# mcap91/SpatialCore

Measured on AMD Instinct MI355X. Metric: genes/sec Moran's I (1000 perms, 1M cells, k=15), higher is better.
Workload: dtype f64

## Files before the change

spatialcore_amd/csrc/sc_moran.hip:

```cpp
#include <math.h>
#include <stdlib.h>

#include <functional>
#include <vector>

#include "sc_permgen.h"


#define MP_PERMS_PER_BLOCK 32

__global__ __launch_bounds__(256) void k_moran_perm(const double *__restrict__ Zt,
                                                    const double *__restrict__ Lt,
                                                    const int32_t *__restrict__ perm,
                                                    double *__restrict__ partial, int64_t n,
                                                    int64_t pstride, int n_perm, int64_t cells_per_split)
{
    const int wave = threadIdx.x >> 6, lane = threadIdx.x & 63;
    const int r = lane >> 3, q = lane & 7;
    const int pbase = blockIdx.y * MP_PERMS_PER_BLOCK + wave * 8;
    if (pbase >= n_perm) return;
    const int p = pbase + r;
    const int pc = p < n_perm ? p : n_perm - 1;
    const int64_t c0 = (int64_t)blockIdx.x * cells_per_split;
    int64_t c1 = c0 + cells_per_split;
// ... 22 lines not shown
        const double2 z4 = Z2[(i + 4) * 8];
        const double2 z5 = Z2[(i + 5) * 8];
        const double2 z6 = Z2[(i + 6) * 8];
        const double2 z7 = Z2[(i + 7) * 8];
        a0x = fma(z0.x, l0.x, a0x); a0y = fma(z0.y, l0.y, a0y);
        a1x = fma(z1.x, l1.x, a1x); a1y = fma(z1.y, l1.y, a1y);
        a0x = fma(z2.x, l2.x, a0x); a0y = fma(z2.y, l2.y, a0y);
        a1x = fma(z3.x, l3.x, a1x); a1y = fma(z3.y, l3.y, a1y);
        a0x = fma(z4.x, l4.x, a0x); a0y = fma(z4.y, l4.y, a0y);
        a1x = fma(z5.x, l5.x, a1x); a1y = fma(z5.y, l5.y, a1y);
        a0x = fma(z6.x, l6.x, a0x); a0y = fma(z6.y, l6.y, a0y);
        a1x = fma(z7.x, l7.x, a1x); a1y = fma(z7.y, l7.y, a1y);
    }
    for (; i < c1; ++i) {
        const double2 l = L2[(int64_t)prow[i] * 8];
        const double2 z = Z2[i * 8];
        a0x = fma(z.x, l.x, a0x);
        a0y = fma(z.y, l.y, a0y);
    }
    if (p < n_perm) {
        double2 *out = reinterpret_cast<double2 *>(partial) +
                       ((int64_t)blockIdx.x * n_perm + p) * 8 + q;
        *out = make_double2(a0x + a1x, a0y + a1y);
    }
}

__global__ __launch_bounds__(256) void k_moran_finalize(const double *__restrict__ partial,
                                                        const double *__restrict__ seff, const double *__restrict__ corr,
                                                        double *__restrict__ sims, double *__restrict__ raw, int n_perm, int splits,
                                                        int64_t n_genes, int64_t g0, int64_t p0)
{
    int t = blockIdx.x * blockDim.x + threadIdx.x;
    int p = t >> 4, slot = t & 15;
    if (p >= n_perm || g0 + slot >= n_genes) return;
    double s = 0.0;
    for (int k = 0; k < splits; ++k) s += partial[((int64_t)k * n_perm + p) * SC_TILE + slot];
    raw[(p0 + p) * n_genes + g0 + slot] = s;
    sims[(p0 + p) * n_genes + g0 + slot] = seff[g0 + slot] * (s - corr[g0 + slot]);
}

__global__ void k_moran_scale(const double *__restrict__ z2, const double *__restrict__ inum, const double *__restrict__ slag,
                              const double *__restrict__ mean, const double *__restrict__ lat, double *__restrict__ seff,
                              double *__restrict__ corr, double *__restrict__ thr, double *__restrict__ I, double n_over_s0,
                              double w, int64_t total)
{
    int64_t g = (int64_t)blockIdx.x * blockDim.x + threadIdx.x;
    if (g >= total) return;
    const bool l = lat[g] != 0.0;
    const double sc = l ? (n_over_s0 / z2[g]) * w : n_over_s0 / z2[g];
    const double co = l ? mean[g] * slag[g] : 0.0;
    const double v = sc * (inum[g] - co);
    seff[g] = sc;
    corr[g] = co;
    I[g] = v;
    thr[g] = l ? inum[g] : v;
}

__global__ __launch_bounds__(256) void k_moran_count(const double *__restrict__ sims, const double *__restrict__ raw,
                                                     const double *__restrict__ thr, const double *__restrict__ lat,
                                                     const double *__restrict__ z2, int n_perm,
                                                     int64_t n_genes, long long *__restrict__ count,
                                                     double *__restrict__ ssum, double *__restrict__ ssq)
{
    __shared__ double sh_a[256], sh_b[256];
    __shared__ int sh_c[256];
    int64_t g = blockIdx.x;
    const double t = thr[g];
    const bool l = lat[g] != 0.0, alive = z2[g] > 0.0;
    double a = 0.0, b = 0.0;
    int cnt = 0;
    for (int p = threadIdx.x; p < n_perm; p += 256) {
        double v = sims[(int64_t)p * n_genes + g];
        const double cv = l ? raw[(int64_t)p * n_genes + g] : v;
        cnt += (alive && cv >= t) ? 1 : 0;
        a += v;
        b += v * v;
    }
    sh_a[threadIdx.x] = a;
    sh_b[threadIdx.x] = b;
    sh_c[threadIdx.x] = cnt;
    __syncthreads();
    for (int s = 128; s > 0; s >>= 1) {
        if ((int)threadIdx.x < s) {
            sh_a[threadIdx.x] += sh_a[threadIdx.x + s];
            sh_b[threadIdx.x] += sh_b[threadIdx.x + s];
            sh_c[threadIdx.x] += sh_c[threadIdx.x + s];
        }
        __syncthreads();
    }
    if (threadIdx.x == 0) {
        count[g] = sh_c[0];
        ssum[g] = sh_a[0];
        ssq[g] = sh_b[0];
    }
}


__global__ void k_moran_centres(const double *__restrict__ mean, const double *__restrict__ lat, double *__restrict__ centre,
                                int64_t total)
{
    const int64_t g = (int64_t)blockIdx.x * blockDim.x + threadIdx.x;
    if (g < total) centre[g] = lat[g] != 0.0 ? 0.0 : mean[g];
}


#define SCORE_WAVES 16
#define SCORE_PRIVATE_WAVES 8

__device__ __forceinline__ double2 lag16_to_double2(uint32_t v) { return make_double2((double)(v & 0xffffu), (double)(v >> 16)); }


template <bool BIG>
__device__ __forceinline__ uint4 score_row(const char *const &Xg, const uint32_t &qoff, int32_t i)
{
    if constexpr (BIG) return *reinterpret_cast<const uint4 *>(Xg + ((uint64_t)(uint32_t)i * 128u + qoff));
    else return *reinterpret_cast<const uint4 *>(Xg + ((uint32_t)i * 128u + qoff));
}

template <int CB>
__device__ __forceinline__ void score_load_idx(int4 (&id)[CB / 4], const int32_t *const &irow, const int64_t &c0, int64_t b, const int64_t &nblk)
{
    const int64_t bb = b < nblk ? b : nblk - 1;
#pragma unroll
    for (int k = 0; k < CB / 4; ++k) id[k] = *reinterpret_cast<const int4 *>(irow + c0 + bb * CB + 4 * k);
}

template <int CB, bool BIG>
__device__ __forceinline__ void score_gather(uint4 (&x)[CB], const int4 (&id)[CB / 4], const char *const &Xg, const uint32_t &qoff)
{
#pragma unroll
    for (int k = 0; k < CB / 4; ++k) {
        x[4 * k + 0] = score_row<BIG>(Xg, qoff, id[k].x);
        x[4 * k + 1] = score_row<BIG>(Xg, qoff, id[k].y);
        x[4 * k + 2] = score_row<BIG>(Xg, qoff, id[k].z);
        x[4 * k + 3] = score_row<BIG>(Xg, qoff, id[k].w);
    }
}

template <int BITS, bool CENTER>
__device__ __forceinline__ void score_fma(const uint32_t (&w)[4], int t, double2 l, const double (&m)[2], double (&acc)[2])
{
    double v0, v1;
    if (BITS == 8) {
        const uint32_t h = w[t >> 1] >> (16 * (t & 1));
        v0 = (double)(h & 0xffu); v1 = (double)((h >> 8) & 0xffu);
    } else if (BITS == 16) { v0 = (double)(w[t] & 0xffffu); v1 = (double)(w[t] >> 16); }
    else if (BITS == 32) { v0 = (double)__uint_as_float(w[2 * t]); v1 = (double)__uint_as_float(w[2 * t + 1]); }
    else { v0 = __hiloint2double((int)w[1], (int)w[0]); v1 = __hiloint2double((int)w[3], (int)w[2]); }
    if constexpr (CENTER) { v0 -= m[0]; v1 -= m[1]; }
    acc[0] = fma(l.x, v0, acc[0]);
    acc[1] = fma(l.y, v1, acc[1]);
}

template <int BITS, int CB, bool BIG, bool L16 = false>
__global__ __launch_bounds__(SCORE_PRIVATE_WAVES * 64) void k_moran_score(
    const uint4 *__restrict__ narrow, const double *__restrict__ Lag, int64_t tile_elems, int tiles16,
    const double *__restrict__ mean, const int32_t *__restrict__ inv, double *__restrict__ partial, int64_t n,
    int64_t pstride, int n_perm, int64_t cells_per_split, int n_splits, int n_groups)
{
    static_assert((BITS == 8 || BITS == 16 || BITS == 32 || BITS == 64) && (CB == 4 || CB == 8), "source width / block size");
    static_assert(!L16 || BITS == 8, "16-bit lag rows belong to the uint8 source");
    constexpr int TG = BITS == 8 ? 8 : BITS == 16 ? 4 : BITS == 32 ? 2 : 1;
    constexpr bool CENTER = BITS == 16 || BITS == 32;
    constexpr int ROW = TG * 8;
    static_assert((CB * ROW) % 64 == 0, "a block's lag rows are loaded by whole wavefront instructions");
    constexpr int NI = CB / 4;
    constexpr int NL = CB * ROW / 64;
    constexpr int CSTEP = 64 / ROW;
    __shared__ double2 lds_lag[SCORE_PRIVATE_WAVES][2][CB * ROW];
    const int wave = threadIdx.x >> 6, lane = threadIdx.x & 63;
    const int r = lane >> 3, q = lane & 7;
    const int lcell0 = lane / ROW, ltile = (lane % ROW) >> 3;
    double2 *lw = &lds_lag[wave][0][0];
    const int pgroups = (n_perm + 7) >> 3;
    const int64_t n_tasks = (int64_t)n_groups * n_splits * pgroups;
    const int64_t worker = (int64_t)blockIdx.x * SCORE_PRIVATE_WAVES + wave, workers = (int64_t)gridDim.x * SCORE_PRIVATE_WAVES;

    for (int64_t task = worker; task < n_tasks; task += workers) {
        const int pg = (int)(task % pgroups);
        const int64_t rest = task / pgroups;
        const int split = (int)(rest % n_splits), grp = (int)(rest / n_splits);
        const int p = pg * 8 + r;
        const int pc = p < n_perm ? p : n_perm - 1;
        const int64_t c0 = (int64_t)split * cells_per_split;
        int64_t c1 = c0 + cells_per_split;
        if (c1 > n) c1 = n;
        const int32_t *irow = inv + (int64_t)pc * pstride;
        const char *Xg = reinterpret_cast<const char *>(narrow + (int64_t)grp * n * 8);
        const uint32_t qoff = (uint32_t)q * 16u;
        const int tiles_left = tiles16 - TG * grp;
        const double *lag_g = Lag + (int64_t)TG * grp * tile_elems;
        const double2 *lsrc = reinterpret_cast<const double2 *>(lag_g + (int64_t)(ltile < tiles_left ? ltile : 0) * tile_elems) + (lane & 7);
        const uint32_t *lag16_g = reinterpret_cast<const uint32_t *>(Lag) + (int64_t)grp * n * ROW;
        const uint32_t *lsrc16 = lag16_g + (lane % ROW);
        double m[CENTER ? TG : 1][2], acc[TG][2];
#pragma unroll
        for (int t = 0; t < TG; ++t) {
            if constexpr (CENTER) {
                const double *mt = mean + (int64_t)(TG * grp + (t < tiles_left ? t : 0)) * SC_TILE + 2 * q;
                m[t][0] = mt[0]; m[t][1] = mt[1];
            }
            acc[t][0] = acc[t][1] = 0.0;
        }
        const int64_t nblk = (c1 - c0) / CB;

        int4 ida[NI], idb[NI];
        double2 lg0, lg1, lg2, lg3;
        uint32_t lh0 = 0, lh1 = 0, lh2 = 0, lh3 = 0;
        uint4 xa[CB], xb[CB];

        auto load_idx = [&](int4 (&id)[NI], int64_t b) { score_load_idx<CB>(id, irow, c0, b, nblk); };
        auto load_lag = [&](int64_t b) {
            const int64_t bb = b < nblk ? b : nblk - 1;
            const int64_t row0 = c0 + bb * CB + lcell0;
            if constexpr (L16) {
                lh0 = lsrc16[row0 * ROW];
                if constexpr (NL > 1) lh1 = lsrc16[(row0 + CSTEP) * ROW];
                if constexpr (NL > 2) { lh2 = lsrc16[(row0 + 2 * CSTEP) * ROW]; lh3 = lsrc16[(row0 + 3 * CSTEP) * ROW]; }
            } else {
                lg0 = lsrc[row0 * 8];
                if constexpr (NL > 1) lg1 = lsrc[(row0 + CSTEP) * 8];
                if constexpr (NL > 2) { lg2 = lsrc[(row0 + 2 * CSTEP) * 8]; lg3 = lsrc[(row0 + 3 * CSTEP) * 8]; }
            }
        };
        auto gather = [&](uint4 (&x)[CB], const int4 (&id)[NI]) { score_gather<CB, BIG>(x, id, Xg, qoff); };
        auto park_lag = [&](int buf) {
            double2 *dst = lw + buf * (CB * ROW) + lane;
            if constexpr (L16) {
                dst[0] = lag16_to_double2(lh0);
                if constexpr (NL > 1) dst[64] = lag16_to_double2(lh1);
                if constexpr (NL > 2) { dst[128] = lag16_to_double2(lh2); dst[192] = lag16_to_double2(lh3); }
            } else {
                dst[0] = lg0;
                if constexpr (NL > 1) dst[64] = lg1;
                if constexpr (NL > 2) { dst[128] = lg2; dst[192] = lg3; }
            }
        };
        auto mul_cell = [&](const uint4 &x, const double2 *lr) {
            const uint32_t w[4] = {x.x, x.y, x.z, x.w};
#pragma unroll
            for (int t = 0; t < TG; ++t) score_fma<BITS, CENTER>(w, t, lr[t * 8], m[CENTER ? t : 0], acc[t]);
        };
        auto multiply = [&](const uint4 (&x)[CB], int buf) {
            const double2 *lr = lw + buf * (CB * ROW) + q;
#pragma unroll
            for (int c = 0; c < CB; ++c) mul_cell(x[c], lr + c * ROW);
        };
        auto stage = [&](const uint4 (&cur)[CB], uint4 (&nxt)[CB], int4 (&id_next)[NI], int64_t b) {
            load_lag(b + 1);
            __builtin_amdgcn_sched_barrier(0);
            gather(nxt, id_next);
            __builtin_amdgcn_sched_barrier(0);
            load_idx(id_next, b + 3);
            __builtin_amdgcn_sched_barrier(0);
            park_lag((int)((b + 1) & 1));
            multiply(cur, (int)(b & 1));
            __builtin_amdgcn_sched_barrier(0);
        };

        if (nblk > 0) {
            load_idx(ida, 0);
            load_lag(0);
            gather(xa, ida);
            load_idx(idb, 1);
            load_idx(ida, 2);
            park_lag(0);
            int64_t b = 0;
            for (; b + 2 <= nblk; b += 2) {
                stage(xa, xb, idb, b);
                stage(xb, xa, ida, b + 1);
            }
            if (b < nblk) stage(xa, xb, idb, b);
        }
        for (int64_t j = c0 + nblk * CB; j < c1; ++j) {
            const uint4 x = score_row<BIG>(Xg, qoff, irow[j]);
            const uint32_t w[4] = {x.x, x.y, x.z, x.w};
#pragma unroll
            for (int t = 0; t < TG; ++t) {
                double2 l;
                if constexpr (L16) l = lag16_to_double2(lag16_g[j * ROW + t * 8 + q]);
                else l = reinterpret_cast<const double2 *>(lag_g + (int64_t)(t < tiles_left ? t : 0) * tile_elems)[j * 8 + q];
                score_fma<BITS, CENTER>(w, t, l, m[CENTER ? t : 0], acc[t]);
            }
        }
        if (p < n_perm) {
            double2 *out = reinterpret_cast<double2 *>(partial) + (((int64_t)grp * n_splits + split) * n_perm + p) * ROW + q;
#pragma unroll
            for (int t = 0; t < TG; ++t) out[t * 8] = make_double2(acc[t][0], acc[t][1]);
        }
    }
}

#define SCORE_SB 16
#define SCORE_WG_MIN_PERMS 24

template <int BITS, int CB, bool BIG, bool L16 = false>
__global__ __launch_bounds__(SCORE_WAVES * 64) void k_moran_score_wg(
    const uint4 *__restrict__ narrow, const double *__restrict__ Lag, int64_t tile_elems, int tiles16,
    const double *__restrict__ mean, const int32_t *__restrict__ inv, double *__restrict__ partial, int64_t n,
    int64_t pstride, int n_perm, int64_t cells_per_split, int n_splits, int n_groups)
{
    static_assert((BITS == 4 || BITS == 8 || BITS == 16 || BITS == 32 || BITS == 64) && (CB == 4 || CB == 8), "source width / block size");
    constexpr bool NIB = BITS == 4;
    constexpr int TG = BITS == 8 ? 8 : BITS == 16 ? 4 : BITS == 32 ? 2 : NIB ? 4 : 1;
    constexpr bool CENTER = BITS == 16 || BITS == 32;
    constexpr int ROW = TG * 8;
    constexpr int NI = CB / 4;
    constexpr int SPS = SCORE_SB / CB;
    constexpr int PIECES = SCORE_SB * ROW;
    static_assert(PIECES <= SCORE_WAVES * 64 && (SCORE_WAVES * 64) % PIECES == 0, "every thread loads one piece");
    __shared__ double2 lds_lag[2][PIECES];
    const int wave = threadIdx.x >> 6, lane = threadIdx.x & 63;
    const int r = lane >> 3, q = lane & 7;
    const int pid = (int)threadIdx.x % PIECES;
    const int lcell = pid / ROW, ltile = (pid % ROW) >> 3;
    const int pchunks = (n_perm + 8 * SCORE_WAVES - 1) / (8 * SCORE_WAVES);
    const int64_t n_tasks = (int64_t)n_groups * n_splits * pchunks;

    for (int64_t task = blockIdx.x; task < n_tasks; task += gridDim.x) {
        const int pch = (int)(task % pchunks);
        const int64_t rest = task / pchunks;
        const int split = (int)(rest % n_splits), grp = (int)(rest / n_splits);
        const int pbase = (pch * SCORE_WAVES + (BITS != 64 ? __builtin_amdgcn_readfirstlane(wave) : wave)) * 8;
        const bool live = pbase < n_perm;
        const int p = pbase + r;
        const int pc = p < n_perm ? p : n_perm - 1;
        const int64_t c0 = (int64_t)split * cells_per_split;
        int64_t c1 = c0 + cells_per_split;
        if (c1 > n) c1 = n;
        const int32_t *irow = inv + (int64_t)pc * pstride;
        const char *Xg = reinterpret_cast<const char *>(narrow + (int64_t)grp * n * 8);
        const uint32_t qoff = (uint32_t)q * 16u;
        const int tiles_left = tiles16 - TG * grp;
        const double *lag_g = Lag + (int64_t)TG * grp * tile_elems;
        const double2 *lsrc = NIB ? reinterpret_cast<const double2 *>(Lag) + (int64_t)grp * n * ROW + (pid % ROW)
                                  : reinterpret_cast<const double2 *>(lag_g + (int64_t)(ltile < tiles_left ? ltile : 0) * tile_elems) + (pid & 7);
        constexpr int LSTRIDE = NIB ? ROW : 8;
        const uint32_t *lag16_g = reinterpret_cast<const uint32_t *>(Lag) + (int64_t)grp * n * ROW;
        const uint32_t *lsrc16 = lag16_g + (pid % ROW);
        double m[CENTER ? TG : 1][2], acc[TG][2];
#pragma unroll
        for (int t = 0; t < TG; ++t) {
            if constexpr (CENTER) {
                const double *mt = mean + (int64_t)(TG * grp + (t < tiles_left ? t : 0)) * SC_TILE + 2 * q;
                m[t][0] = mt[0]; m[t][1] = mt[1];
            }
            acc[t][0] = acc[t][1] = 0.0;
        }
        uint32_t ai[NIB ? 32 : 1];
#pragma unroll
        for (int k2 = 0; k2 < (NIB ? 32 : 1); ++k2) ai[k2] = 0u;
        const int64_t nsb = (c1 - c0) / SCORE_SB;
        const int64_t nblk = nsb * SPS;

        double2 lg;
        uint32_t lh = 0;
        uint4 xa[CB], xb[CB];
        auto park = [&](int buf) {
            if constexpr (L16) lds_lag[buf][pid] = lag16_to_double2(lh);
            else lds_lag[buf][pid] = lg;
        };

        auto load_idx = [&](int4 (&id)[NI], int64_t b) { score_load_idx<CB>(id, irow, c0, b, nblk); };
        auto load_lag = [&](int64_t sb) {
            const int64_t ss = sb < nsb ? sb : nsb - 1;
            if constexpr (L16) lh = lsrc16[(c0 + ss * SCORE_SB + lcell) * ROW];
            else lg = lsrc[(c0 + ss * SCORE_SB + lcell) * LSTRIDE];
        };
        auto gather = [&](uint4 (&x)[CB], const int4 (&id)[NI]) { score_gather<CB, BIG>(x, id, Xg, qoff); };
        auto mul_cell = [&](const uint4 &x, const double2 *lr) {
            const uint32_t w[4] = {x.x, x.y, x.z, x.w};
            if constexpr (NIB) {
#pragma unroll
                for (int t = 0; t < 4; ++t) {
                    const uint4 sp = *reinterpret_cast<const uint4 *>(&lr[t * 8]);
                    const uint32_t sw[4] = {sp.x, sp.y, sp.z, sp.w};
#pragma unroll
                    for (int e = 0; e < 8; ++e)
                        ai[t * 8 + e] += __umul24((w[t] >> (4 * e)) & 15u, (sw[e >> 1] >> (16 * (e & 1))) & 0xffffu);
                }
                return;
            }
#pragma unroll
            for (int t = 0; t < TG; ++t) score_fma<BITS, CENTER>(w, t, lr[t * 8], m[CENTER ? t : 0], acc[t]);
        };
        auto stage = [&](const uint4 (&cur)[CB], uint4 (&nxt)[CB], int4 (&id_next)[NI], int64_t sb, int k) {
            if (k == 0) load_lag(sb + 1);
            __builtin_amdgcn_sched_barrier(0);
            gather(nxt, id_next);
            __builtin_amdgcn_sched_barrier(0);
            load_idx(id_next, sb * SPS + k + 1 + SPS);
            __builtin_amdgcn_sched_barrier(0);
            const double2 *lr = &lds_lag[sb & 1][k * CB * ROW + q];
#pragma unroll
            for (int c = 0; c < CB; ++c) {
                mul_cell(cur[c], lr + c * ROW);
                if constexpr (NIB) __builtin_amdgcn_sched_barrier(0);
            }
            __builtin_amdgcn_sched_barrier(0);
            if (k == SPS - 1) {
                park((int)((sb + 1) & 1));
                __syncthreads();
            }
        };

        if (BITS != 64 && nsb > 0 && !live) {
            load_lag(0);
            park(0);
            __syncthreads();
            for (int64_t sb = 0; sb < nsb; ++sb) {
                load_lag(sb + 1);
                park((int)((sb + 1) & 1));
                __syncthreads();
            }
        } else if (nsb > 0) {
            int4 id0[NI], id1[NI], id2[NI], id3[NI];
            load_lag(0);
            load_idx(id3, 0);
            gather(xa, id3);
            load_idx(id0, 1);
            load_idx(id1, 2);
            if constexpr (SPS == 4) { load_idx(id2, 3); load_idx(id3, 4); }
            park(0);
            __syncthreads();
            for (int64_t sb = 0; sb < nsb; ++sb) {
                stage(xa, xb, id0, sb, 0);
                stage(xb, xa, id1, sb, 1);
                if constexpr (SPS == 4) {
                    stage(xa, xb, id2, sb, 2);
                    stage(xb, xa, id3, sb, 3);
                }
            }
        }
        if (live) {
            for (int64_t j = c0 + nsb * SCORE_SB; j < c1; ++j) {
                const uint4 x = score_row<BIG>(Xg, qoff, irow[j]);
                const uint32_t w[4] = {x.x, x.y, x.z, x.w};
                if constexpr (NIB) {
                    const uint4 *srow = reinterpret_cast<const uint4 *>(Lag) + ((int64_t)grp * n + j) * ROW + q;
#pragma unroll
                    for (int t = 0; t < 4; ++t) {
                        const uint4 sp = srow[t * 8];
                        const uint32_t sw[4] = {sp.x, sp.y, sp.z, sp.w};
#pragma unroll
                        for (int e = 0; e < 8; ++e)
                            ai[t * 8 + e] += __umul24((w[t] >> (4 * e)) & 15u, (sw[e >> 1] >> (16 * (e & 1))) & 0xffffu);
                    }
                    continue;
                }
#pragma unroll
                for (int t = 0; t < TG; ++t) {
                    double2 l;
                    if constexpr (L16) l = lag16_to_double2(lag16_g[j * ROW + t * 8 + q]);
                    else l = reinterpret_cast<const double2 *>(lag_g + (int64_t)(t < tiles_left ? t : 0) * tile_elems)[j * 8 + q];
                    score_fma<BITS, CENTER>(w, t, l, m[CENTER ? t : 0], acc[t]);
                }
            }
            if (p < n_perm) {
                if constexpr (NIB) {
                    double2 *out = reinterpret_cast<double2 *>(partial + ((((int64_t)grp * n_splits + split) * n_perm + p) * 256 + q * 8));
#pragma unroll
                    for (int t = 0; t < 4; ++t)
#pragma unroll
                        for (int e2 = 0; e2 < 4; ++e2)
                            out[t * 32 + e2] = make_double2((double)ai[t * 8 + 2 * e2], (double)ai[t * 8 + 2 * e2 + 1]);
                } else {
                double2 *out = reinterpret_cast<double2 *>(partial) + (((int64_t)grp * n_splits + split) * n_perm + p) * ROW + q;
#pragma unroll
                for (int t = 0; t < TG; ++t) out[t * 8] = make_double2(acc[t][0], acc[t][1]);
                }
            }
        }
    }
}

template <int GP>
__global__ __launch_bounds__(256) void k_moran_finalize_groups(const double *__restrict__ partial,
                                                               const double *__restrict__ seff,
                                                               const double *__restrict__ corr,
                                                               double *__restrict__ sims, double *__restrict__ raw, int n_perm,
                                                               int splits, int64_t n_genes, int64_t p0)
{
    const int t = blockIdx.x * blockDim.x + threadIdx.x;
    const int p = t / GP, slot = t % GP;
    const int64_t g = GP * (int64_t)blockIdx.y + slot;
    if (p >= n_perm || g >= n_genes) return;
    const double *pt = partial + (int64_t)blockIdx.y * splits * n_perm * GP;
    double s = 0.0;
    for (int k = 0; k < splits; ++k) s += pt[((int64_t)k * n_perm + p) * GP + slot];
    raw[(p0 + p) * n_genes + g] = s;
    sims[(p0 + p) * n_genes + g] = seff[g] * (s - corr[g]);
}

static int64_t score_cells_per_split(int64_t n)
{
    int64_t cps = align_up64(ceil_div64(n, 512), 8);
    return cps < 2048 ? 2048 : cps;
}

static int pick_splits(int64_t n, int n_perm_tiles, int64_t *cells_per_split)
{
    int64_t want = ceil_div64(2048, n_perm_tiles > 0 ? n_perm_tiles : 1);
    if (want < 1) want = 1;
    if (want > 256) want = 256;
    int64_t cps = align_up64(ceil_div64(n, want), 8);
    if (cps < 2048) cps = 2048;
    *cells_per_split = cps;
    return (int)ceil_div64(n, cps);
}

static int moran_check(sc_ctx *c, int64_t n_perm, const double *I_out)
{
    SC_REQUIRE(c && I_out, SC_ERR_INVALID, "sc_moran: null pointer");
    SC_REQUIRE(n_perm >= 0 && n_perm <= (1 << 24), SC_ERR_INVALID, "sc_moran: n_perm=%lld out of range",
               (long long)n_perm);
    SC_HIP(hipSetDevice(c->device));
    SC_REQUIRE(c->e_n > 0, SC_ERR_STATE, "sc_moran: no expression loaded");
    SC_REQUIRE(c->g_n > 0, SC_ERR_STATE, "sc_moran: no graph set");
    SC_REQUIRE(c->g_n == c->e_n, SC_ERR_INVALID, "sc_moran: graph has %lld rows but expression has %lld cells",
               (long long)c->g_n, (long long)c->e_n);
    return SC_OK;
}

__global__ __launch_bounds__(256) void k_lag_f32rows(const int64_t *__restrict__ indptr, const int32_t *__restrict__ indices,
                                                     const double *__restrict__ w, const uint4 *__restrict__ narrow,
                                                     const double *__restrict__ centre, double *__restrict__ Lag, int64_t n,
                                                     int tiles16, const double *__restrict__ unit,
                                                     const int32_t *__restrict__ order)
{
    const int64_t per_xcd = (int64_t)(gridDim.x >> 3);
    const int64_t blk = (int64_t)(blockIdx.x & 7) * per_xcd + (blockIdx.x >> 3);
    const int64_t t = blk * blockDim.x + threadIdx.x;
    const int64_t pos = t >> 3;
    const int q = (int)(t & 7);
    if (pos >= n) return;
    const int64_t i = order ? order[pos] : pos;
    const int grp = blockIdx.y;
    const int tiles_left = tiles16 - 2 * grp;
    const uint4 *Xg = narrow + (int64_t)grp * n * 8;
    double cen[4];
    bool un[4];
#pragma unroll
    for (int k = 0; k < 4; ++k) {
        const int64_t g = (int64_t)(2 * grp + ((k >> 1) < tiles_left ? (k >> 1) : 0)) * SC_TILE + 2 * q + (k & 1);
        cen[k] = centre[g];
        un[k] = unit && unit[g] != 0.0;
    }
    const int64_t e0 = indptr[i], e1 = indptr[i + 1];
    double s[4] = {0.0, 0.0, 0.0, 0.0};
    for (int64_t e = e0; e < e1; ++e) {
        const uint4 v = Xg[(int64_t)indices[e] * 8 + q];
        const double ww = w[e];
        const double z[4] = {(double)__uint_as_float(v.x) - cen[0], (double)__uint_as_float(v.y) - cen[1],
                             (double)__uint_as_float(v.z) - cen[2], (double)__uint_as_float(v.w) - cen[3]};
#pragma unroll
        for (int k = 0; k < 4; ++k) s[k] = __dadd_rn(s[k], __dmul_rn(un[k] ? 1.0 : ww, z[k]));
    }
    reinterpret_cast<double2 *>(Lag + (int64_t)(2 * grp) * n * SC_TILE)[i * 8 + q] = make_double2(s[0], s[1]);
    if (tiles_left > 1) reinterpret_cast<double2 *>(Lag + (int64_t)(2 * grp + 1) * n * SC_TILE)[i * 8 + q] = make_double2(s[2], s[3]);
}

#define LAG8_CELLS_PER_BLOCK 4096

__global__ __launch_bounds__(256) void k_lag_u8(const long long *__restrict__ indptr, const int32_t *__restrict__ indices,
                                                const uint4 *__restrict__ narrow, const int32_t *__restrict__ order, int64_t n,
                                                int tiles16, int64_t tile_elems, double *__restrict__ Lag,
                                                uint32_t *__restrict__ Lag16 ,
                                                double *__restrict__ partial , int chunks)
{
    __shared__ double shT[128], shS[128];
    const int grp = blockIdx.y;
    const int64_t per_xcd = (int64_t)(gridDim.x >> 3);
    const int64_t chunk = (int64_t)(blockIdx.x & 7) * per_xcd + (blockIdx.x >> 3);
    const int q = threadIdx.x & 7, row = threadIdx.x >> 3;
    if (threadIdx.x < 128) { shT[threadIdx.x] = 0.0; shS[threadIdx.x] = 0.0; }
    __syncthreads();
    const uint4 *Xg = narrow + (int64_t)grp * n * 8;
    const int tiles_left = tiles16 - 8 * grp;
    double accT[16], accS[16];
#pragma unroll
    for (int b = 0; b < 16; ++b) accT[b] = accS[b] = 0.0;
    const int64_t p0 = chunk * LAG8_CELLS_PER_BLOCK;
    if (chunk < chunks) {
        for (int it = 0; it < LAG8_CELLS_PER_BLOCK / 32; ++it) {
            const int64_t pos = p0 + it * 32 + row;
            if (pos >= n) break;
            const int64_t cell = order ? order[pos] : pos;
            const uint4 own = Xg[cell * 8 + q];
            uint32_t lo[4] = {0u, 0u, 0u, 0u}, hi[4] = {0u, 0u, 0u, 0u};
            for (long long e = indptr[cell]; e < indptr[cell + 1]; ++e) {
                const uint4 v = Xg[(int64_t)indices[e] * 8 + q];
                const uint32_t w[4] = {v.x, v.y, v.z, v.w};
#pragma unroll
                for (int k = 0; k < 4; ++k) { lo[k] += w[k] & 0x00ff00ffu; hi[k] += (w[k] >> 8) & 0x00ff00ffu; }
            }
            const uint32_t xo[4] = {own.x, own.y, own.z, own.w};
#pragma unroll
            for (int t = 0; t < 8; ++t) {
                const int k = t >> 1, sh = 16 * (t & 1);
                const double s0 = (double)((lo[k] >> sh) & 0xffffu), s1 = (double)((hi[k] >> sh) & 0xffffu);
                const double x0 = (double)((xo[k] >> sh) & 0xffu), x1 = (double)((xo[k] >> (sh + 8)) & 0xffu);
                if (Lag16) Lag16[((int64_t)grp * n + cell) * 64 + t * 8 + q] = ((lo[k] >> sh) & 0xffffu) | (((hi[k] >> sh) & 0xffffu) << 16);
                else if (t < tiles_left)
                    reinterpret_cast<double2 *>(Lag + (int64_t)(8 * grp + t) * tile_elems)[cell * 8 + q] = make_double2(s0, s1);
                accS[2 * t] += s0; accS[2 * t + 1] += s1;
                accT[2 * t] = fma(x0, s0, accT[2 * t]); accT[2 * t + 1] = fma(x1, s1, accT[2 * t + 1]);
            }
        }
    }
#pragma unroll
    for (int t = 0; t < 8; ++t)
#pragma unroll
        for (int e = 0; e < 2; ++e) {
            atomicAdd(&shT[t * 16 + 2 * q + e], accT[2 * t + e]);
            atomicAdd(&shS[t * 16 + 2 * q + e], accS[2 * t + e]);
        }
    __syncthreads();
    if (threadIdx.x < 128 && chunk < chunks) {
        const int t = threadIdx.x >> 4, slot = threadIdx.x & 15;
        if (t < tiles_left) {
            const int64_t tile = 8 * grp + t;
            partial[((int64_t)tile * chunks + chunk) * SC_TILE + slot] = shT[threadIdx.x];
// ... 368 lines not shown
        const int64_t tasks = (int64_t)groups * splits * ((cnt + 8 * SCORE_WAVES - 1) / (8 * SCORE_WAVES));
        if (wgs > tasks) wgs = (int)tasks;
        hipLaunchKernelGGL((k_moran_score_wg<BITS, CB, BIG, L16>), dim3((unsigned)wgs), dim3(SCORE_WAVES * 64), 0, c->stream, rows,
                           c->Lag.as<double>(), (int64_t)c->e_n * SC_TILE, (int)c->e_tiles, c->g_meanc.as<double>(),
                           c->inv.as<int32_t>() + p0 * c->p_stride, partial, c->e_n, c->p_stride, cnt, cps,
                           splits, groups);
        return;
    }
    if constexpr (BITS != 4)
    hipLaunchKernelGGL((k_moran_score<BITS, CB, BIG, L16>), dim3((unsigned)(wgs * (SCORE_WAVES / SCORE_PRIVATE_WAVES))),
                       dim3(SCORE_PRIVATE_WAVES * 64), 0, c->stream, rows,
                       c->Lag.as<double>(), (int64_t)c->e_n * SC_TILE, (int)c->e_tiles, c->g_meanc.as<double>(),
                       c->inv.as<int32_t>() + p0 * c->p_stride, partial, c->e_n, c->p_stride, cnt, cps,
                       splits, groups);
}

static int moran_perm_range(sc_ctx *c, int64_t p0, int64_t p1, int bits, bool invert_here)
{
    const int64_t n = c->e_n, G = c->e_genes, T = c->e_tiles;
    const size_t tile_elems = (size_t)n * SC_TILE;
    const int cnt = (int)(p1 - p0);
    if (cnt <= 0) return SC_OK;
    c->last_source_bits = bits ? bits : 64;
    if (bits) {
        const bool big = n >= ((int64_t)1 << 25);
        SC_REQUIRE(!big || bits == 64, SC_ERR_STATE, "internal: %lld cells need the 64-bit-address scoring kernel", (long long)n);
        if (invert_here) SC_TRY(invert_rows(c, p0, p1, c->stream));
        const int GP = bits == 4 ? 256 : bits == 8 ? 128 : bits == 16 ? 64 : bits == 32 ? 32 : 16;
        const int groups = bits == 4 ? c->nib_groups : (int)ceil_div64(T * SC_TILE, GP);
        const int64_t cps = score_cells_per_split(n);
        const int splits = (int)ceil_div64(n, cps);
        if (c->n_cus <= 0) {
            hipDeviceProp_t prop;
            SC_HIP(hipGetDeviceProperties(&prop, c->device));
            c->n_cus = prop.multiProcessorCount;
        }
        int wgs = c->n_cus - (c->score_leave_cus > 0 && c->score_leave_cus < c->n_cus ? c->score_leave_cus : 0);
        const int64_t tasks = (int64_t)groups * splits * ((cnt + 7) / 8);
        if ((int64_t)wgs * SCORE_WAVES > tasks) wgs = (int)ceil_div64(tasks, SCORE_WAVES);
        double *partial = nullptr;
        SC_TRY(moran_ring_slice(c, &partial));
        {
            KernelTimerScope ts(c, SC_K_MORAN_PERM);
            if (bits == 4) launch_score<4, 4, false>(c, wgs, c->X32.as<uint4>(), partial, p0, cnt, cps, splits, groups);
            else if (bits == 8 && c->lag_u16) launch_score<8, 4, false, true>(c, wgs, c->X32.as<uint4>(), partial, p0, cnt, cps, splits, groups);
            else if (bits == 8) launch_score<8, 4, false>(c, wgs, c->X32.as<uint4>(), partial, p0, cnt, cps, splits, groups);
            else if (bits == 16) launch_score<16, 4, false>(c, wgs, c->X32.as<uint4>(), partial, p0, cnt, cps, splits, groups);
            else if (bits == 32) launch_score<32, 4, false>(c, wgs, c->X32.as<uint4>(), partial, p0, cnt, cps, splits, groups);
            else if (!big) launch_score<64, 8, false>(c, wgs, c->Z.as<uint4>(), partial, p0, cnt, cps, splits, groups);
            else launch_score<64, 8, true>(c, wgs, c->Z.as<uint4>(), partial, p0, cnt, cps, splits, groups);
        }
        SC_TRY(moran_ring_scored(c));
        if (bits == 4) {
            hipLaunchKernelGGL(k_moran_finalize_nib, dim3((unsigned)ceil_div64((int64_t)cnt * G, 256)), dim3(256), 0, c->stream_out,
                               partial, c->g_seff.as<double>(), c->g_corr.as<double>(), c->nib_map.as<int32_t>(),
                               c->sims.as<double>(), c->sims_raw.as<double>(), cnt, splits, G, p0);
            return moran_ring_finalised(c);
        }
        const dim3 fgrid((unsigned)ceil_div64((int64_t)cnt * GP, 256), (unsigned)groups);
        auto fin = bits == 8 ? k_moran_finalize_groups<128> : bits == 16 ? k_moran_finalize_groups<64>
                 : bits == 32 ? k_moran_finalize_groups<32> : k_moran_finalize_groups<16>;
        hipLaunchKernelGGL(fin, fgrid, dim3(256), 0, c->stream_out, partial, c->g_seff.as<double>(),
                           c->g_corr.as<double>(), c->sims.as<double>(), c->sims_raw.as<double>(), cnt, splits, G, p0);
        return moran_ring_finalised(c);
    }
    const int ptiles = (int)ceil_div64(cnt, MP_PERMS_PER_BLOCK);
    int64_t cps = 0;
    const int splits = pick_splits(n, ptiles, &cps);
    for (int64_t t = 0; t < T; ++t) {
        double *partial = nullptr;
        SC_TRY(moran_ring_slice(c, &partial));
        {
            KernelTimerScope ts(c, SC_K_MORAN_PERM);
            hipLaunchKernelGGL(k_moran_perm, dim3((unsigned)splits, (unsigned)ptiles), dim3(256), 0, c->stream,
                               c->Z.as<double>() + t * tile_elems, c->Lag.as<double>() + t * tile_elems,
                               c->perm.as<int32_t>() + p0 * c->p_stride, partial, n, c->p_stride,
                               cnt, cps);
        }
        SC_TRY(moran_ring_scored(c));
        hipLaunchKernelGGL(k_moran_finalize, dim3((unsigned)ceil_div64((int64_t)cnt * SC_TILE, 256)), dim3(256), 0,
                           c->stream_out, partial, c->g_seff.as<double>(), c->g_corr.as<double>(),
                           c->sims.as<double>(), c->sims_raw.as<double>(), cnt, splits, G, t * SC_TILE, p0);
        SC_TRY(moran_ring_finalised(c));
    }
    return SC_OK;
}

static int moran_alloc_sims(sc_ctx *c, int64_t n_perm)
{
    const size_t bytes = sizeof(double) * (size_t)(c->e_tiles * SC_TILE) * (size_t)(n_perm > 0 ? n_perm : 1);
    SC_TRY(c->sims.ensure(bytes, &c->mem));
    SC_TRY(c->sims_raw.ensure(bytes, &c->mem));
    return SC_OK;
}

static int moran_finish(sc_ctx *c, int64_t n_perm, double *I_out, double *sims_out, int64_t *count_ge_out,
                        double *sim_sum_out, double *sim_sumsq_out)
{
    const int64_t G = c->e_genes;
    if (n_perm > 0) {
        SC_TRY(c->counts.ensure(sizeof(long long) * (size_t)G, &c->mem));
        SC_TRY(c->sim_sum.ensure(sizeof(double) * (size_t)G, &c->mem));
        SC_TRY(c->sim_sumsq.ensure(sizeof(double) * (size_t)G, &c->mem));
        SC_TRY(moran_ring_join(c));
        hipLaunchKernelGGL(k_moran_count, dim3((unsigned)G), dim3(256), 0, c->stream, c->sims.as<double>(),
                           c->sims_raw.as<double>(), c->g_thr.as<double>(), c->g_lat.as<double>(), c->g_z2.as<double>(),
                           (int)n_perm, G, c->counts.as<long long>(), c->sim_sum.as<double>(),
                           c->sim_sumsq.as<double>());
        SC_HIP(hipGetLastError());
        if (sims_out)
            SC_HIP(hipMemcpyAsync(sims_out, c->sims.p, sizeof(double) * (size_t)n_perm * (size_t)G,
                                  hipMemcpyDeviceToHost, c->stream));
        if (count_ge_out)
            SC_HIP(hipMemcpyAsync(count_ge_out, c->counts.p, sizeof(int64_t) * (size_t)G, hipMemcpyDeviceToHost,
                                  c->stream));
        if (sim_sum_out)
            SC_HIP(hipMemcpyAsync(sim_sum_out, c->sim_sum.p, sizeof(double) * (size_t)G, hipMemcpyDeviceToHost,
                                  c->stream));
        if (sim_sumsq_out)
            SC_HIP(hipMemcpyAsync(sim_sumsq_out, c->sim_sumsq.p, sizeof(double) * (size_t)G,
                                  hipMemcpyDeviceToHost, c->stream));
    }
    SC_HIP(hipMemcpyAsync(I_out, c->g_I.p, sizeof(double) * (size_t)G, hipMemcpyDeviceToHost, c->stream));
    SC_HIP(hipStreamSynchronize(c->stream));
    c->ring.launches = 0;
    return SC_OK;
}

extern "C" int sc_moran(sc_ctx *c, int64_t n_perm, double *I_out, double *sims_out, int64_t *count_ge_out,
                        double *sim_sum_out, double *sim_sumsq_out)
{
    SC_TRY(moran_check(c, n_perm, I_out));
    if (n_perm > 0) {
        SC_REQUIRE(c->p_count >= n_perm, SC_ERR_STATE, "sc_moran: permutation table holds %lld rows, need %lld",
                   (long long)c->p_count, (long long)n_perm);
        SC_REQUIRE(c->p_n == c->e_n, SC_ERR_INVALID, "sc_moran: permutation length %lld != n_cells %lld",
                   (long long)c->p_n, (long long)c->e_n);
    }
    const bool inverse_suffices = n_perm > 0 && c->perm_bijective && c->inv_rows_valid >= n_perm;
    if (n_perm > 0 && !inverse_suffices) SC_TRY(sc_perm_forward_ensure(c));
    bool bijective = true;
    SC_TRY(sc_perm_table_is_bijective(c, n_perm, &bijective));
    SC_TRY(moran_prepare(c, n_perm < PERM_CHUNK ? n_perm : PERM_CHUNK, n_perm <= 0 || bijective));
    SC_TRY(moran_alloc_sims(c, n_perm));
    const int bits = bijective ? c->narrow_bits : 0;
    for (int64_t p0 = 0; p0 < n_perm; p0 += PERM_CHUNK) {
        const int64_t p1 = p0 + PERM_CHUNK < n_perm ? p0 + PERM_CHUNK : n_perm;
        SC_TRY(moran_perm_range(c, p0, p1, bits, bits != 0 && p1 > c->inv_rows_valid));
        if (bits != 0 && p1 > c->inv_rows_valid) c->inv_rows_valid = p1;
    }
    return moran_finish(c, n_perm, I_out, sims_out, count_ge_out, sim_sum_out, sim_sumsq_out);
}

#define SCORE_RESERVED_CUS 112
static int moran_seeded_once(sc_ctx *c, uint64_t *state6, int64_t n_perm, double *I_out, double *sims_out,
                             int64_t *count_ge_out, double *sim_sum_out, double *sim_sumsq_out, PermPipe *begun)
{
    SC_REQUIRE(state6, SC_ERR_INVALID, "sc_moran_seeded: null state");
    SC_TRY(moran_check(c, n_perm, I_out));
    SC_REQUIRE(n_perm >= 1, SC_ERR_INVALID, "sc_moran_seeded: n_perm must be >= 1 (use sc_moran for n_perm = 0)");
    const int64_t n = c->e_n;
    SC_TRY(moran_alloc_sims(c, n_perm));
    const bool inverse_only = permgen_can_swap_inverse(n);
    int bits = 64;
    auto prepare_early = [&]() -> int { return moran_prepare_early(c); };
    auto prepare = [&]() -> int {
        SC_TRY(moran_prepare(c, n_perm < PERM_CHUNK ? n_perm : PERM_CHUNK, true));
        bits = c->narrow_bits;
        if (c->score_leave_cus > 8) c->score_leave_cus = bits == 8 ? SCORE_RESERVED_CUS : bits == 16 ? 96 : 64;
        return SC_OK;
    };
    auto score = [&](int64_t p0, int64_t p1) -> int {
        const int keep = c->score_leave_cus;
        if (keep > 8) {
            const int tail_prev = keep < 32 ? keep : 32, tail_last = 8;
            if (p1 == n_perm) c->score_leave_cus = tail_last;
            else if (n_perm > 3 * PERM_CHUNK && n_perm - p1 < PIPE_TAIL_TOTAL) c->score_leave_cus = tail_prev;
        }
        const int rc = moran_perm_range(c, p0, p1, bits, false);
        c->score_leave_cus = keep;
        return rc;
    };
    if (begun) SC_TRY(pipe_consume(c, *begun, state6, prepare_early, prepare, score));
    else SC_TRY(sc_perm_pipeline(c, state6, n, n_perm, inverse_only ? 1 : 2, PIPE_AHEAD, prepare_early, prepare, score));
    return moran_finish(c, n_perm, I_out, sims_out, count_ge_out, sim_sum_out, sim_sumsq_out);
}

static int moran_seeded_streams(sc_ctx *c, uint64_t *state6, int64_t n_perm, double *I_out, double *sims_out,
                                int64_t *count_ge_out, double *sim_sum_out, double *sim_sumsq_out, PermPipe *begun = nullptr)
{
    c->score_leave_cus = c && c->e_n > 0 && permgen_is_block_parallel(c, c->e_n) ? SCORE_RESERVED_CUS : 8;
    const int rc = moran_seeded_once(c, state6, n_perm, I_out, sims_out, count_ge_out, sim_sum_out, sim_sumsq_out, begun);
    c->score_leave_cus = 0;
    return rc;
}

extern "C" int sc_moran_seeded(sc_ctx *c, uint64_t *state6, int64_t n_perm, double *I_out, double *sims_out,
                               int64_t *count_ge_out, double *sim_sum_out, double *sim_sumsq_out)
{
    SC_REQUIRE(c, SC_ERR_INVALID, "sc_moran_seeded: null context");
    return permgen_rerun_on_failure(
        c, [&]() { return moran_seeded_streams(c, state6, n_perm, I_out, sims_out, count_ge_out, sim_sum_out, sim_sumsq_out); },
        nullptr);
}

extern "C" int sc_moran_seeded_begin(sc_ctx *c, const uint64_t *state6, int64_t n_cells, int64_t n_perm, int64_t ahead_chunks)
{
    SC_REQUIRE(c && state6, SC_ERR_INVALID, "sc_moran_seeded_begin: null pointer");
    SC_REQUIRE(n_perm >= 1 && n_perm <= (1 << 24), SC_ERR_INVALID, "sc_moran_seeded_begin: n_perm=%lld out of range", (long long)n_perm);
    SC_HIP(hipSetDevice(c->device));
    sc_perm_pipe_abort(c);
    auto pp = std::make_unique<PermPipe>();
    const int64_t ahead_n = ahead_chunks <= 0 ? (int64_t)1 << 40 : (ahead_chunks < 2 ? 2 : ahead_chunks);
    SC_TRY(pipe_begin(c, state6, n_cells, n_perm, permgen_can_swap_inverse(n_cells) ? 1 : 2, PIPE_AHEAD, *pp, ahead_n));
    c->pipe = std::move(pp);
    return SC_OK;
}

extern "C" int sc_moran_seeded_abort(sc_ctx *c)
{
    SC_REQUIRE(c, SC_ERR_INVALID, "null context");
    SC_HIP(hipSetDevice(c->device));
    sc_perm_pipe_abort(c);
    return SC_OK;
}

extern "C" int sc_moran_seeded_finish(sc_ctx *c, uint64_t *state6, double *I_out, double *sims_out, int64_t *count_ge_out,
                                      double *sim_sum_out, double *sim_sumsq_out)
{
    SC_REQUIRE(c && state6, SC_ERR_INVALID, "sc_moran_seeded_finish: null pointer");
    SC_REQUIRE(c->pipe, SC_ERR_STATE, "sc_moran_seeded_finish: no job begun (sc_moran_seeded_begin)");
    SC_HIP(hipSetDevice(c->device));
    std::unique_ptr<PermPipe> pp = std::move(c->pipe);
    const int64_t n_perm = pp->n_perm;
    auto attempt = [&]() -> int {
        if (!pp) return moran_seeded_streams(c, state6, n_perm, I_out, sims_out, count_ge_out, sim_sum_out, sim_sumsq_out);
        SC_REQUIRE(pp->n == c->e_n, SC_ERR_INVALID, "sc_moran_seeded_finish: the job was begun for %lld cells, the expression has %lld",
                   (long long)pp->n, (long long)c->e_n);
        return moran_seeded_streams(c, state6, n_perm, I_out, sims_out, count_ge_out, sim_sum_out, sim_sumsq_out, pp.get());
    };
    auto drop = [&]() -> int {
        pipe_drain(c, *pp);
        for (int k = 0; k < 6; ++k) state6[k] = pp->state0[k];
        pp.reset();
        return SC_OK;
    };
    const int rc = permgen_rerun_on_failure(c, attempt, drop);
    if (pp) pipe_drain(c, *pp);
    return rc;
}
```

Measured before the change: 3366.

## Score uint8 source with udot4 integer dot products over byte-plane lag

For the uint8 source with 16-bit lag rows, the lag is parked in LDS as byte planes (low and high bytes, interleaved across 4 cells). Gene bytes are transposed with v_perm so udot4 can accumulate 4 cells at a time into 32-bit integer accumulators, replacing per-element f64 FMAs. The result is rebuilt as lo + 256*hi in double at the end. This also shrinks LDS use and raises the reserved CU count for the 8-bit path, at the risk of uint32 overflow on long splits and added permute overhead.

```diff
diff --git a/spatialcore_amd/csrc/sc_moran.hip b/spatialcore_amd/csrc/sc_moran.hip
--- a/spatialcore_amd/csrc/sc_moran.hip
+++ b/spatialcore_amd/csrc/sc_moran.hip
@@ -198,6 +198,37 @@
     acc[1] = fma(l.y, v1, acc[1]);
 }
 
+
+__device__ __forceinline__ void score_transpose4(uint32_t a, uint32_t b, uint32_t c, uint32_t d, uint32_t (&o)[4])
+{
+    const uint32_t ab0 = __builtin_amdgcn_perm(b, a, 0x05010400u), ab1 = __builtin_amdgcn_perm(b, a, 0x07030602u);
+    const uint32_t cd0 = __builtin_amdgcn_perm(d, c, 0x05010400u), cd1 = __builtin_amdgcn_perm(d, c, 0x07030602u);
+    o[0] = __builtin_amdgcn_perm(cd0, ab0, 0x05040100u);
+    o[1] = __builtin_amdgcn_perm(cd0, ab0, 0x07060302u);
+    o[2] = __builtin_amdgcn_perm(cd1, ab1, 0x05040100u);
+    o[3] = __builtin_amdgcn_perm(cd1, ab1, 0x07060302u);
+}
+
+__device__ __forceinline__ void score_dot_block(const uint4 (&x)[4], const uint4 *sp, uint32_t (&lo)[16], uint32_t (&hi)[16])
+{
+    const uint32_t w[4][4] = {{x[0].x, x[0].y, x[0].z, x[0].w}, {x[1].x, x[1].y, x[1].z, x[1].w},
+                              {x[2].x, x[2].y, x[2].z, x[2].w}, {x[3].x, x[3].y, x[3].z, x[3].w}};
+#pragma unroll
+    for (int k = 0; k < 4; ++k) {
+        uint32_t o[4];
+        score_transpose4(w[0][k], w[1][k], w[2][k], w[3][k], o);
+#pragma unroll
+        for (int h = 0; h < 2; ++h) {
+            const uint4 s = sp[(2 * k + h) * 8];
+            const int g = 4 * k + 2 * h;
+            lo[g] = __builtin_amdgcn_udot4(o[2 * h], s.x, lo[g], false);
+            hi[g] = __builtin_amdgcn_udot4(o[2 * h], s.y, hi[g], false);
+            lo[g + 1] = __builtin_amdgcn_udot4(o[2 * h + 1], s.z, lo[g + 1], false);
+            hi[g + 1] = __builtin_amdgcn_udot4(o[2 * h + 1], s.w, hi[g + 1], false);
+        }
+    }
+}
+
 template <int BITS, int CB, bool BIG, bool L16 = false>
 __global__ __launch_bounds__(SCORE_PRIVATE_WAVES * 64) void k_moran_score(
     const uint4 *__restrict__ narrow, const double *__restrict__ Lag, int64_t tile_elems, int tiles16,
@@ -355,7 +386,8 @@
     constexpr int SPS = SCORE_SB / CB;
     constexpr int PIECES = SCORE_SB * ROW;
     static_assert(PIECES <= SCORE_WAVES * 64 && (SCORE_WAVES * 64) % PIECES == 0, "every thread loads one piece");
-    __shared__ double2 lds_lag[2][PIECES];
+    constexpr bool PLANES = BITS == 8 && CB == 4 && !BIG && L16;
+    __shared__ double2 lds_lag[2][PLANES ? SCORE_SB / 4 * ROW : PIECES];
     const int wave = threadIdx.x >> 6, lane = threadIdx.x & 63;
     const int r = lane >> 3, q = lane & 7;
     const int pid = (int)threadIdx.x % PIECES;
@@ -396,6 +428,9 @@
         uint32_t ai[NIB ? 32 : 1];
 #pragma unroll
         for (int k2 = 0; k2 < (NIB ? 32 : 1); ++k2) ai[k2] = 0u;
+        uint32_t plo[PLANES ? 16 : 1], phi[PLANES ? 16 : 1];
+#pragma unroll
+        for (int k2 = 0; k2 < (PLANES ? 16 : 1); ++k2) plo[k2] = phi[k2] = 0u;
         const int64_t nsb = (c1 - c0) / SCORE_SB;
         const int64_t nblk = nsb * SPS;
 
@@ -403,6 +438,11 @@
         uint32_t lh = 0;
         uint4 xa[CB], xb[CB];
         auto park = [&](int buf) {
+            if constexpr (PLANES) {
+                unsigned char *dst = reinterpret_cast<unsigned char *>(&lds_lag[buf][(lcell >> 2) * ROW + (pid % ROW)]) + (lcell & 3);
+                dst[0] = (unsigned char)lh; dst[4] = (unsigned char)(lh >> 8);
+                dst[8] = (unsigned char)(lh >> 16); dst[12] = (unsigned char)(lh >> 24);
+            } else
             if constexpr (L16) lds_lag[buf][pid] = lag16_to_double2(lh);
             else lds_lag[buf][pid] = lg;
         };
@@ -437,9 +477,10 @@
             __builtin_amdgcn_sched_barrier(0);
             load_idx(id_next, sb * SPS + k + 1 + SPS);
             __builtin_amdgcn_sched_barrier(0);
-            const double2 *lr = &lds_lag[sb & 1][k * CB * ROW + q];
-#pragma unroll
-            for (int c = 0; c < CB; ++c) {
+            const double2 *lr = &lds_lag[sb & 1][(PLANES ? k * ROW : k * CB * ROW) + q];
+            if constexpr (PLANES) score_dot_block(cur, reinterpret_cast<const uint4 *>(lr), plo, phi);
+#pragma unroll
+            for (int c = 0; c < (PLANES ? 0 : CB); ++c) {
                 mul_cell(cur[c], lr + c * ROW);
                 if constexpr (NIB) __builtin_amdgcn_sched_barrier(0);
             }
@@ -479,6 +520,20 @@
             }
         }
         if (live) {
+            if constexpr (PLANES) {
+#pragma clang loop vectorize(disable) interleave(disable) unroll(disable)
+                for (int64_t j = c0 + nsb * SCORE_SB; j < c1; ++j) {
+                    const uint4 x = score_row<BIG>(Xg, qoff, irow[j]);
+                    const uint32_t w[4] = {x.x, x.y, x.z, x.w};
+#pragma unroll
+                    for (int t = 0; t < TG; ++t) {
+                        const uint32_t s = lag16_g[j * ROW + t * 8 + q], h = w[t >> 1] >> (16 * (t & 1));
+                        const uint32_t x0 = h & 0xffu, x1 = (h >> 8) & 0xffu;
+                        plo[2 * t] += __umul24(x0, s & 0xffu); phi[2 * t] += __umul24(x0, (s >> 8) & 0xffu);
+                        plo[2 * t + 1] += __umul24(x1, (s >> 16) & 0xffu); phi[2 * t + 1] += __umul24(x1, s >> 24);
+                    }
+                }
+            } else
             for (int64_t j = c0 + nsb * SCORE_SB; j < c1; ++j) {
                 const uint4 x = score_row<BIG>(Xg, qoff, irow[j]);
                 const uint32_t w[4] = {x.x, x.y, x.z, x.w};
@@ -513,7 +568,11 @@
                 } else {
                 double2 *out = reinterpret_cast<double2 *>(partial) + (((int64_t)grp * n_splits + split) * n_perm + p) * ROW + q;
 #pragma unroll
-                for (int t = 0; t < TG; ++t) out[t * 8] = make_double2(acc[t][0], acc[t][1]);
+                for (int t = 0; t < TG; ++t) {
+                    if constexpr (PLANES) out[t * 8] = make_double2((double)plo[2 * t] + 256.0 * (double)phi[2 * t],
+                                                                    (double)plo[2 * t + 1] + 256.0 * (double)phi[2 * t + 1]);
+                    else out[t * 8] = make_double2(acc[t][0], acc[t][1]);
+                }
                 }
             }
         }
@@ -1188,7 +1247,7 @@
     return moran_finish(c, n_perm, I_out, sims_out, count_ge_out, sim_sum_out, sim_sumsq_out);
 }
 
-#define SCORE_RESERVED_CUS 112
+#define SCORE_RESERVED_CUS 128
 static int moran_seeded_once(sc_ctx *c, uint64_t *state6, int64_t n_perm, double *I_out, double *sims_out,
                              int64_t *count_ge_out, double *sim_sum_out, double *sim_sumsq_out, PermPipe *begun)
 {
```

Result: faster. 3486, median of 6 (+3.6%).
